# lcp29/trimesh-ray-optix

Hardware: AMD Instinct MI355X
Metric: Mrays/s closest-hit, 1M-tri mesh, 1024^2 ray batch (higher is better)
Workload: dtype f32; 1 GPU; C5(i): icosphere(8)+displacement seed 0, 1310720 tris; 1024x1024 pinhole rays per GPU; intersects_closest (stream_compaction=False); rays_per_gpu=1048576, rays_total=1048576, triangles=1310720, parallelism=ray-sharded x1, BVH replicated, warmup_steps_done=360, bvh_depth=30, bvh_bytes=104857568

## Files before the change

trimesh-ray-optix_amd/csrc/kernels_direct.inc:

```
template <bool C, bool DEEP = false> struct tr_word { typedef uint64_t T; };
template <> struct tr_word<true, false> { typedef uint32_t T; };

constexpr bool TR_STREAM_QN = true;
template <int Q> constexpr bool TR_STREAM_COLD = Q != TR_Q_CLOSEST;
template <int Q, int K, bool STATS, bool COMPACT = false, bool UNI = false, bool DEEP = false>
__device__ __forceinline__ void wave_traverse(const tr_bvh_view& b, tr_ray& r, bool go,
                                              tr_result& res, tr_topk<K>& top, tr_counters* cnt,
                                              const tr_ring ring) {
    tr_result_init(res);
    if (Q == TR_Q_LOCATION) top.init();
    typedef typename tr_word<COMPACT, DEEP>::T W;
    tr_state_t<W> fs;
    tr_state_init(fs);
    if (!go) fs.node = -1;
    while (!tr_done(fs)) {
        tr_fused_step<Q, K, STATS, COMPACT, W, UNI, true>(b, r, fs, res, top, cnt, ring);
        TR_CONVERGE();
        tr_fused_step<Q, K, STATS, COMPACT, W, UNI, false>(b, r, fs, res, top, cnt, ring);
        TR_CONVERGE();
    }
}

constexpr uint32_t TR_STEAL_EVERY = 3u;
constexpr uint32_t TR_STEAL_EARLY = 4u;
constexpr int TR_STEAL_IDLE = 1;
__device__ __forceinline__ int lane_rank(unsigned long long mask) {
    return (int)__builtin_amdgcn_mbcnt_hi((unsigned)(mask >> 32), __builtin_amdgcn_mbcnt_lo((unsigned)mask, 0u));
}

template <int Q, bool STATS, bool COMPACT, bool DEEP = false, bool QN = false>
__device__ __forceinline__ bool wave_traverse_steal(const tr_bvh_view& b, tr_ray& r, bool go,
                                                    tr_result& res, tr_counters* cnt,
                                                    const tr_ring ring, int32_t* wl, int lane,
                                                    uint32_t steal_min, bool& lost) {
    constexpr bool PLAIN = QN;
    typedef typename std::conditional<PLAIN, tr_plaina_w, typename tr_word<COMPACT, DEEP>::T>::type W;
    lost = false;
    tr_result_init(res);
    tr_topk<1> top;
    tr_state_t<W> fs;
    const tr_aring ar = tr_aring_of(ring);
    (void)ar;
    if constexpr (PLAIN) tr_state_init(fs, tr_addr_start(ring));
    else tr_state_init(fs);
    if (!go) fs.node = -1;
    auto trip_step = [&](auto test_tag) {
        constexpr bool TEST = decltype(test_tag)::value;
        if (!tr_done(fs)) tr_fused_step<Q, 1, STATS, COMPACT, W, false, TEST, QN>(b, r, fs, res, top, cnt, ring);
    };
    int owner = lane;
    bool split = false;
    uint32_t trip = 0;
    if (steal_min & 0x8000u) {
        steal_min &= 0x7fffu;
        const unsigned long long act = __ballot(go);
        if (act != 0ull) {
            const int l0 = (int)__builtin_ctzll(act);
            const float ax = __shfl(r.dx, l0), ay = __shfl(r.dy, l0), az = __shfl(r.dz, l0);
            const float bx = __shfl(r.ox, l0) - r.ox, by = __shfl(r.oy, l0) - r.oy, bz = __shfl(r.oz, l0) - r.oz;
            const float dd = ax * r.dx + ay * r.dy + az * r.dz;
            const float n0 = ax * ax + ay * ay + az * az, n1 = r.dx * r.dx + r.dy * r.dy + r.dz * r.dz;
            const float ex = 65535.f * b.frame.scale[0], ey = 65535.f * b.frame.scale[1], ez = 65535.f * b.frame.scale[2];
            const bool alike = dd > 0.f && dd * dd >= 0.998f * n0 * n1 && bx * bx + by * by + bz * bz <= 1e-4f * (ex * ex + ey * ey + ez * ez);
            if (4 * __popcll(__ballot(go && alike)) < 3 * __popcll(act) && steal_min > TR_STEAL_EARLY) steal_min = TR_STEAL_EARLY;
        }
    }
    typedef __attribute__((address_space(3))) volatile int32_t lds_i32;
    typedef __attribute__((address_space(3))) volatile unsigned long long lds_u64;
    lds_i32* const lw = (lds_i32*)wl;
    lds_i32* const list = lw;
    lds_i32* const xnode = lw + 64;
    lds_i32* const xdepth = lw + 128;
    int32_t* const xflags = wl + 128;
    if constexpr (PLAIN) xdepth[lane] = 0;
    constexpr int ACC = 192;
    int32_t* sum = wl + ACC;
    unsigned long long* keys = reinterpret_cast<unsigned long long*>(wl + ACC);
    lds_i32* const vsum = lw + ACC;
    lds_u64* const vkeys = (lds_u64*)(lw + ACC);
    lds_i32* const vslots = lw + ACC + 128;
    auto deposit = [&]() {
        if constexpr (PLAIN) {
            if (tr_addr_lost(fs.sa)) atomicOr(&xflags[owner], 0x100);
        }
        if (Q == TR_Q_COUNT) {
            if (res.count) atomicAdd(&sum[owner], res.count);
        } else if (Q == TR_Q_ANY) {
            if (res.best_face >= 0) vsum[owner] = 1;
        } else {
            const bool have = res.best_slot >= 0;
            const unsigned long long key = ((unsigned long long)(__float_as_uint(res.best_t) & 0x7fffffffu) << 32) |
                                           (unsigned)res.best_face;
            if (have) atomicMin(&keys[owner], key);
            __builtin_amdgcn_wave_barrier();
            if (have && vkeys[owner] == key) vslots[owner] = res.best_slot;
        }
    };
    uint32_t k0 = 0;
    if constexpr (PLAIN) {
        bool l0 = false, l1 = false;
        int32_t c0 = 0, c1 = 0;
        while (trip < steal_min) {
            l0 = false; l1 = false;
            if (fs.node >= 0) tr_descent_step<Q, STATS, COMPACT>(b, r, fs, res, cnt, ring, l0, l1, c0, c1);
            TR_CONVERGE();
            trip++;
            if (TR_WAVE_ANY(l0 || l1) || !TR_WAVE_ANY(fs.node >= 0)) break;
        }
        fs.p0 = l0 ? ~c0 : (l1 ? ~c1 : -1);
        fs.p1 = (l0 && l1) ? ~c1 : -1;
        if (trip & 1u) {
            trip_step(std::false_type{});
            TR_CONVERGE();
            trip++;
        }
        k0 = trip == 0u ? 0u : ((trip - 1u) & TR_STEAL_EVERY) + 1u;
        trip -= k0;
    }
    for (;;) {
#pragma unroll 1
        for (uint32_t k = k0; k <= TR_STEAL_EVERY; k += 2) {
            trip_step(std::true_type{});
            TR_CONVERGE();
            trip_step(std::false_type{});
            TR_CONVERGE();
        }
        k0 = 0;
        trip += (TR_STEAL_EVERY / 2u + 1u) * 2u;
        if (split) {
            if (Q == TR_Q_ANY) {
                if (res.best_face >= 0) vsum[owner] = 1;
                __builtin_amdgcn_wave_barrier();
                if (vsum[owner] != 0 && !tr_done(fs)) { fs.node = -1; fs.p0 = -1; fs.p1 = -1; fs.p2 = -1; }
            } else if (Q == TR_Q_CLOSEST || Q == TR_Q_FIRST) {
                const bool have = res.best_slot >= 0;
                const unsigned long long mine = ((unsigned long long)(__float_as_uint(res.best_t) & 0x7fffffffu) << 32) |
                                                (unsigned)(res.best_face < 0 ? 0x7fffffff : res.best_face);
                if (have) atomicMin(&keys[owner], mine);
                __builtin_amdgcn_wave_barrier();
                const unsigned long long k = vkeys[owner];
                if (have && k == mine) vslots[owner] = res.best_slot;
                if (k < mine) {
                    tr_set_best_t(res, __uint_as_float((unsigned)(k >> 32)));
                    res.best_face = (int32_t)(unsigned)k;
                    res.best_slot = -1;
                }
            }
        }
        const bool done = tr_done(fs);
        const unsigned long long idle = __ballot(done);
        if (idle == ~0ull) break;
        if (__popcll(idle) >= TR_STEAL_IDLE && trip >= steal_min) {
            uint32_t bot = 0;
            bool has_far;
            if constexpr (PLAIN) {
                bot = (uint32_t)xdepth[lane] & 0xffu;
                has_far = tr_addr_can_give(ar, fs.sa, bot);
            } else {
                has_far = (fs.trail & fs.owned) != 0;
            }
            const bool can_give = !done && has_far;
            const unsigned long long donors = __ballot(can_give);
            const int ni = __popcll(idle), nd = __popcll(donors);
            const int np = ni < nd ? ni : nd;
            if (np > 0) {
                if (!split) {
                    if (Q == TR_Q_COUNT || Q == TR_Q_ANY) vsum[lane] = 0;
                    else vkeys[lane] = ~0ull;
                    split = true;
                    __builtin_amdgcn_wave_barrier();
                }
                const int drank = lane_rank(donors), irank = lane_rank(idle);
                const bool give = can_give && drank < np;
                int gnode = 0, gdepth = 0;
                (void)gdepth;
                if constexpr (PLAIN) {
                    if (give) {
                        gnode = tr_addr_give(ar, fs.sa, bot);
                        list[drank] = lane; xnode[lane] = gnode;
                        atomicAdd(&xflags[lane], 1);
                    }
                } else if (give) {
                    uint32_t j;
                    gnode = tr_ring_get(ring, tr_bottom_slot<W>(fs.trail, fs.owned, j));
                    gdepth = (int32_t)(j + 1);
                    list[drank] = lane; xnode[lane] = gnode; xdepth[lane] = gdepth;
                    fs.trail &= ~(W(1) << j);
                }
                __builtin_amdgcn_wave_barrier();
                const bool take = done && irank < np;
                const int src = take ? list[irank] : lane;
                if (take) {
                    deposit();
                    tr_result_init(res);
                }
                r.ox = __shfl(r.ox, src); r.oy = __shfl(r.oy, src); r.oz = __shfl(r.oz, src);
                r.dx = __shfl(r.dx, src); r.dy = __shfl(r.dy, src); r.dz = __shfl(r.dz, src);
                r.ix = __shfl(r.ix, src); r.iy = __shfl(r.iy, src); r.iz = __shfl(r.iz, src);
                r.kd = __shfl(r.kd, src);
                r.sel_n = (uint32_t)__shfl((int)r.sel_n, src); r.sel_f = (uint32_t)__shfl((int)r.sel_f, src); r.sel_z = (uint32_t)__shfl((int)r.sel_z, src);
                if constexpr (QN) {
                    r.qax = __shfl(r.qax, src); r.qay = __shfl(r.qay, src); r.qaz = __shfl(r.qaz, src);
                    r.qnx = __shfl(r.qnx, src); r.qny = __shfl(r.qny, src); r.qnz = __shfl(r.qnz, src);
                    r.qfx = __shfl(r.qfx, src); r.qfy = __shfl(r.qfy, src); r.qfz = __shfl(r.qfz, src);
                    r.qaz2 = r.qaz;
                }
                const int own2 = __shfl(owner, src);
                const float bt = __shfl(res.best_t, src);
                if (take) {
                    owner = own2;
                    if constexpr (PLAIN) {
                        tr_state_init(fs, tr_addr_bottom(ar, fs.sa));
                        atomicAnd(&xflags[lane], 0x100);
                    } else {
                        tr_state_init(fs);
                        fs.depth = (uint32_t)xdepth[src];
                    }
                    fs.node = xnode[src];
                    tr_set_best_t(res, bt);
                }
                __builtin_amdgcn_wave_barrier();
            }
        }
    }
    if (split) {
        deposit();
        __builtin_amdgcn_wave_barrier();
        if (Q == TR_Q_COUNT) {
            res.count = vsum[lane];
        } else if (Q == TR_Q_ANY) {
            res.best_face = vsum[lane] ? 0 : -1;
        } else {
            const unsigned long long k = vkeys[lane];
            tr_result_init(res);
            if (k != ~0ull) {
                tr_set_best_t(res, __uint_as_float((unsigned)(k >> 32)));
                res.best_face = (int32_t)(unsigned)k;
                res.best_slot = vslots[lane];
            }
        }
        if constexpr (PLAIN) lost = (xdepth[lane] & 0x100) != 0;
    } else if constexpr (PLAIN) {
        lost = tr_addr_lost(fs.sa);
    }
    return split;
}

template <int Q, bool STATS, bool COMPACT = false, bool UNI = false, bool DEEP = false>
__device__ __forceinline__ void process_ray(const tr_bvh_view& b, const RayFetch& rf,
                                            const QueryOut& out, int64_t i, bool in_range,
                                            tr_counters* cnt, const tr_ring ring) {
    float o[3] = {0.f, 0.f, 0.f}, d[3] = {0.f, 0.f, 0.f};
    if (in_range) fetch_ray(rf, i, o, d);
    tr_ray r;
    const bool valid = tr_ray_setup_a(r, b.frame, o[0], o[1], o[2], d[0], d[1], d[2]) && in_range;
    tr_result res;
    if (Q == TR_Q_LOCATION) {
        tr_topk<0> top;
        top.ent = out.hits + (in_range ? i : 0) * out.cap;
        top.tris = b.tris;
        top.cap = out.cap;
        if (b.num_tris >= 2) {
            wave_traverse<Q, 0, STATS, COMPACT, UNI, DEEP>(b, r, valid, res, top, cnt, ring);
        } else {
            top.init();
            brute_one<Q>(b, r, valid, res);
            if (res.count) top.insert(res.best_t, res.best_face, 0);
        }
    } else {
        tr_topk<1> top;
        if (b.num_tris >= 2) wave_traverse<Q, 1, STATS, COMPACT, UNI, DEEP>(b, r, valid, res, top, cnt, ring);
        else brute_one<Q>(b, r, valid, res);
    }
    if (in_range) write_result<Q>(b, out, i, r, res);
}

template <int Q>
__device__ __attribute__((noinline)) tr_result retraverse_lost(const tr_node* nodes, const tr_link* links, const tr_tri* tris,
                                                               float b0, float b1, float b2, float s0, float s1, float s2,
                                                               float ox, float oy, float oz, float dx, float dy, float dz,
                                                               float best_t, int32_t best_face, int32_t best_slot) {
    tr_bvh_view v;
    v.nodes = nodes; v.links = links; v.tris = tris; v.num_tris = 2; v.qnodes = nullptr; v.frame_dev = nullptr;
    v.frame.base[0] = b0; v.frame.base[1] = b1; v.frame.base[2] = b2;
    v.frame.scale[0] = s0; v.frame.scale[1] = s1; v.frame.scale[2] = s2;
    tr_result res;
    res.best_t = best_t; res.best_face = best_face; res.best_slot = best_slot; res.count = 0;
    tr_ray r;
    if (tr_ray_setup_a(r, v.frame, ox, oy, oz, dx, dy, dz)) {
        tr_topk<1> top;
        tr_counters* nc = nullptr;
        tr_traverse_more<Q, 1, false>(v, r, res, top, nc);
    }
    return res;
}

template <int Q, bool STATS, bool COMPACT, bool DEEP = false, bool QN = false>
__device__ __forceinline__ void process_ray_steal(const tr_bvh_view& b, const RayFetch& rf,
                                                  const QueryOut& out, int64_t i, bool in_range,
                                                  tr_counters* cnt, const tr_ring ring, int32_t* wl,
                                                  uint32_t steal_min) {
    float o[3] = {0.f, 0.f, 0.f}, d[3] = {0.f, 0.f, 0.f};
    if (in_range) fetch_ray(rf, i, o, d);
    tr_ray r;
    const bool valid = tr_ray_setup_q(r, b.frame, o[0], o[1], o[2], d[0], d[1], d[2]) && in_range;
    tr_result res;
    bool split = false, lost = false;
    if (b.num_tris >= 2) split = wave_traverse_steal<Q, STATS, COMPACT, DEEP, QN>(b, r, valid, res, cnt, ring, wl, (int)(threadIdx.x & 63), steal_min, lost);
    else brute_one<Q>(b, r, valid, res);
    if (split && in_range) {
        fetch_ray(rf, i, o, d);
        tr_ray_setup_a(r, b.frame, o[0], o[1], o[2], d[0], d[1], d[2]);
    }
    if constexpr (QN) {
        lost = lost && valid;
        if (__builtin_expect(TR_WAVE_ANY(lost), 0)) {
            if (lost) {
                fetch_ray(rf, i, o, d);
                res = retraverse_lost<Q>(b.nodes, b.links, b.tris, b.frame.base[0], b.frame.base[1], b.frame.base[2],
                                         b.frame.scale[0], b.frame.scale[1], b.frame.scale[2], o[0], o[1], o[2], d[0], d[1], d[2],
                                         res.best_t, res.best_face, res.best_slot);
            }
        }
    }
    if (in_range) write_result<Q>(b, out, i, r, res);
}

template <int Q, int K, bool STATS, bool COMPACT, bool DEEP = false>
__device__ __forceinline__ void wave_traverse_unordered(const tr_bvh_view& b, tr_ray& r, bool go,
                                                        tr_result& res, tr_topk<K>& top, tr_counters* cnt,
                                                        const tr_ring ring, const tr_leafq lq, int leaf_min) {
    typedef typename tr_word<COMPACT, DEEP>::T W;
    tr_result_init(res);
    if (Q == TR_Q_LOCATION) top.init();
    tr_ustate_t<W> st;
    tr_ustate_init(st);
    if (!go) st.node = -1;
    for (;;) {
        const bool can_node = tr_ucan_node(st);
        const unsigned long long mn = __ballot(can_node), ml = __ballot(st.nq > 0);
        if ((mn | ml) == 0ull) break;
        const bool parked = st.node >= 0 && !can_node;
        const bool leaf_phase = mn == 0ull || __ballot(parked) != 0ull || (int)__popcll(ml) >= (int)leaf_min;
        tr_unord_step<Q, K, STATS, COMPACT, W>(b, r, can_node, leaf_phase, st, res, top, cnt, ring, lq);
        TR_CONVERGE();
    }
}

template <int Q, bool STATS, bool COMPACT, bool DEEP = false>
__device__ __forceinline__ int wave_count_unordered_steal(const tr_bvh_view& b, tr_ray& r, bool go, tr_counters* cnt,
                                                          const tr_ring ring, const tr_leafq lq, int leaf_min,
                                                          int lane, uint32_t steal_min) {
    typedef typename tr_word<COMPACT, DEEP>::T W;
    tr_result res;
    tr_result_init(res);
    tr_topk<1> top;
    tr_ustate_t<W> st;
    tr_ustate_init(st);
    if (!go) st.node = -1;
    int owner = lane;
    int acc = 0;
    uint32_t trip = 0;
    auto hand_in = [&](bool want) {
        unsigned long long m = __ballot(want && res.count != 0);
        while (m != 0ull) {
            const int t = (int)__builtin_ctzll(m);
            const int o = __builtin_amdgcn_readlane(owner, t), c = __builtin_amdgcn_readlane(res.count, t);
            if (lane == o) acc += c;
            m &= m - 1ull;
        }
        if (want) res.count = 0;
    };
    for (;;) {
        bool live = true;
#pragma unroll 1
        for (int k = 0; k < 4 && live; k++) {
            const bool can_node = tr_ucan_node(st);
            const unsigned long long mn = __ballot(can_node), ml = __ballot(st.nq > 0);
            live = (mn | ml) != 0ull;
            if (live) {
                const bool parked = st.node >= 0 && !can_node;
                const bool leaf_phase = mn == 0ull || __ballot(parked) != 0ull || (int)__popcll(ml) >= (int)leaf_min;
                tr_unord_step<Q, 1, STATS, COMPACT, W>(b, r, can_node, leaf_phase, st, res, top, cnt, ring, lq);
            }
            TR_CONVERGE();
        }
        trip += 4;
        const bool done = tr_udone(st);
        const unsigned long long idle = __ballot(done);
        if (idle == ~0ull) break;
        if (idle == 0ull) continue;
        const W cand = st.trail & st.owned;
        const bool can_give = !done && cand != 0 && trip >= steal_min;
        const unsigned long long donors = __ballot(can_give);
        const int ni = __popcll(idle), nd = __popcll(donors);
        const int np = ni < nd ? ni : nd;
        if (np == 0) continue;
        const int drank = lane_rank(donors), irank = lane_rank(idle);
        const bool give = can_give && drank < np;
        const bool take = done && irank < np;
        const unsigned long long givers = __ballot(give);
        const int tgt = give ? drank : 63 - lane_rank(~givers);
        const int list = __builtin_amdgcn_ds_permute(tgt << 2, lane);
        const int pick = __shfl(list, irank & 63);
        const int src = take ? pick : lane;
// ... 409 lines not shown
```

trimesh-ray-optix_amd/csrc/tr_bvh.h:

```cpp
#pragma once
#include <type_traits>
#include "tr_math.h"
#include "../../include/triro_hip.h"

struct alignas(16) tr_f4 {
    float x, y, z, w;
};
struct alignas(16) tr_i4 {
    int32_t x, y, z, w;
};

struct alignas(64) tr_node {
    float box0[6];
    float box1[6];
    int32_t c0, c1;
    int32_t parent;
    int32_t sibling;
};
static_assert(sizeof(tr_node) == 64, "node must be 64 B");
TR_HD void tr_node_set_box(float* box, const float* lo, const float* hi) {
    box[0] = lo[0]; box[1] = lo[1]; box[2] = lo[2]; box[3] = hi[2]; box[4] = hi[0]; box[5] = hi[1];
}

struct alignas(8) tr_link {
// ... 516 lines not shown
        uint32_t j = 0;
        int32_t far = -1;
        if (tr_pop_far(ring, st.trail, st.owned, j, far)) {
            st.node = far;
        } else {
            int32_t node = st.node;
            uint32_t depth = st.depth;
            while (depth > j + 1) {
                node = parent;
                const tr_link l = b.links[node];
                parent = l.parent; sibling = l.sibling;
                depth--;
                if (STATS) cnt->climbs++;
            }
            st.node = sibling;
        }
        st.depth = j + 1;
    }
}

template <int Q, int K, bool STATS>
TR_HD void tr_leaf_step(const tr_bvh_view& b, const tr_ray& r, tr_state& st, tr_result& res,
                        tr_topk<K>& top, tr_counters* cnt) {
    const int32_t q0 = st.p0, q1 = st.p1;
    tr_counters* nc = nullptr;
    const bool any1 = TR_WAVE_ANY(q1 >= 0);
    const tr_tri t0 = tr_load_tri<false>(b, q0 >= 0 ? q0 : 0, nc);
    tr_tri t1 = t0;
    if (any1) t1 = tr_load_tri<false>(b, q1 >= 0 ? q1 : 0, nc);
    if (STATS && q0 >= 0) cnt->tris++;
    bool fin = tr_fold_leaf<Q, K>(q0 >= 0, r, t0, q0, res, top, st.pe);
    fin = tr_drain_exact<Q, K>(b, r, st.pe, res, top) || fin;
    if (any1) {
        const bool live = q1 >= 0 && !fin;
        if (STATS && live) cnt->tris++;
        fin = tr_fold_leaf<Q, K>(live, r, t1, q1, res, top, st.pe) || fin;
        fin = tr_drain_exact<Q, K>(b, r, st.pe, res, top) || fin;
    }
    st.p0 = -1; st.p1 = -1;
    if (Q == TR_Q_ANY && fin) st.node = -1;
}

TR_HD void tr_qnode_slabs_contract(const tr_ray& r, const tr_qframe& f, const tr_i4& w0, const tr_i4& w1,
                                   float& tn0, float& tf0, float& tn1, float& tf1) {
    const uint32_t q0 = (uint32_t)w0.x, q1 = (uint32_t)w0.y, q2 = (uint32_t)w0.z, q3 = (uint32_t)w0.w;
    const uint32_t q4 = (uint32_t)w1.x, q5 = (uint32_t)w1.y;
    const float sx = f.scale[0], sy = f.scale[1], sz = f.scale[2], bx = f.base[0], by = f.base[1], bz = f.base[2];
    tr_slab(r, tr_qdecode(q0 & 0xffffu, sx, bx), tr_qdecode(q0 >> 16, sy, by), tr_qdecode(q1 & 0xffffu, sz, bz),
            tr_qdecode(q2 & 0xffffu, sx, bx), tr_qdecode(q2 >> 16, sy, by), tr_qdecode(q1 >> 16, sz, bz), tn0, tf0);
    tr_slab(r, tr_qdecode(q3 & 0xffffu, sx, bx), tr_qdecode(q3 >> 16, sy, by), tr_qdecode(q4 & 0xffffu, sz, bz),
            tr_qdecode(q5 & 0xffffu, sx, bx), tr_qdecode(q5 >> 16, sy, by), tr_qdecode(q4 >> 16, sz, bz), tn1, tf1);
}

TR_HD void tr_qnode_slabs(const tr_ray& r, const tr_qframe& f, const tr_i4& w0, const tr_i4& w1,
                          float& tn0, float& tf0, float& tn1, float& tf1) {
#if defined(__HIP_DEVICE_COMPILE__)
    const uint32_t q0 = (uint32_t)w0.x, q1 = (uint32_t)w0.y, q2 = (uint32_t)w0.z, q3 = (uint32_t)w0.w;
    const uint32_t q4 = (uint32_t)w1.x, q5 = (uint32_t)w1.y;
    typedef float tr_v2 __attribute__((ext_vector_type(2)));
    const tr_v2 axy = {r.qax, r.qay}, azz = {r.qaz, r.qaz2};
    const tr_v2 nxy = {r.qnx, r.qny}, fxy = {r.qfx, r.qfy}, bz = {r.qnz, r.qfz};
#define TR_UNPK(w) tr_v2{(float)((w) & 0xffffu), (float)((w) >> 16)}
    {
        const uint32_t pn = __builtin_amdgcn_perm(q2, q0, r.sel_n), pf = __builtin_amdgcn_perm(q2, q0, r.sel_f);
        const uint32_t zz = __builtin_amdgcn_perm(q1, q1, r.sel_z);
        const tr_v2 a = __builtin_elementwise_fma(TR_UNPK(pn), axy, nxy);
        const tr_v2 c = __builtin_elementwise_fma(TR_UNPK(pf), axy, fxy);
        const tr_v2 b = __builtin_elementwise_fma(TR_UNPK(zz), azz, bz);
        tn0 = fmaxf(fmaxf(a.x, a.y), b.x);
        tf0 = fminf(fminf(c.x, c.y), b.y);
    }
    {
        const uint32_t pn = __builtin_amdgcn_perm(q5, q3, r.sel_n), pf = __builtin_amdgcn_perm(q5, q3, r.sel_f);
        const uint32_t zz = __builtin_amdgcn_perm(q4, q4, r.sel_z);
        const tr_v2 a = __builtin_elementwise_fma(TR_UNPK(pn), axy, nxy);
        const tr_v2 c = __builtin_elementwise_fma(TR_UNPK(pf), axy, fxy);
        const tr_v2 b = __builtin_elementwise_fma(TR_UNPK(zz), azz, bz);
        tn1 = fmaxf(fmaxf(a.x, a.y), b.x);
        tf1 = fminf(fminf(c.x, c.y), b.y);
    }
#undef TR_UNPK
#else
    (void)f;
    const bool nx = r.ix < 0.f, ny = r.iy < 0.f, nz = r.iz < 0.f;
    const uint32_t q[6] = {(uint32_t)w0.x, (uint32_t)w0.y, (uint32_t)w0.z, (uint32_t)w0.w, (uint32_t)w1.x, (uint32_t)w1.y};
    float tn[2], tf[2];
    for (int c = 0; c < 2; c++) {
        const uint32_t lox = q[3 * c] & 0xffffu, loy = q[3 * c] >> 16, loz = q[3 * c + 1] & 0xffffu;
        const uint32_t hiz = q[3 * c + 1] >> 16, hix = q[3 * c + 2] & 0xffffu, hiy = q[3 * c + 2] >> 16;
        const float ax = fmaf((float)(nx ? hix : lox), r.qax, r.qnx), ay = fmaf((float)(ny ? hiy : loy), r.qay, r.qny);
        const float az = fmaf((float)(nz ? hiz : loz), r.qaz, r.qnz);
        const float cx = fmaf((float)(nx ? lox : hix), r.qax, r.qfx), cy = fmaf((float)(ny ? loy : hiy), r.qay, r.qfy);
        const float cz = fmaf((float)(nz ? loz : hiz), r.qaz, r.qfz);
        tn[c] = fmaxf(fmaxf(ax, ay), az);
        tf[c] = fminf(fminf(cx, cy), cz);
    }
    tn0 = tn[0]; tf0 = tf[0]; tn1 = tn[1]; tf1 = tf[1];
#endif
}

template <bool STATS>
TR_HD int32_t tr_climb(const tr_bvh_view& b, int32_t node, uint32_t depth, uint32_t j, tr_counters* cnt) {
    tr_link l = b.links[node];
    if (STATS) cnt->climbs++;
    while (depth > j + 1) {
        node = l.parent;
        l = b.links[node];
        depth--;
        if (STATS) cnt->climbs++;
    }
    return l.sibling;
}

struct tr_rec_f { tr_f4 n0, n1, n2, n3; };
struct tr_rec_q { tr_i4 w0, w1; };
TR_HD void tr_rec_slabs(const tr_bvh_view&, const tr_ray& r, const tr_rec_f& n, float& tn0, float& tf0, float& tn1, float& tf1) {
    tr_node_slabs(r, n.n0, n.n1, n.n2, tn0, tf0, tn1, tf1);
}
TR_HD void tr_rec_slabs(const tr_bvh_view& b, const tr_ray& r, const tr_rec_q& n, float& tn0, float& tf0, float& tn1, float& tf1) {
    tr_qnode_slabs(r, b.frame, n.w0, n.w1, tn0, tf0, tn1, tf1);
}
TR_HD void tr_rec_children(const tr_rec_f& n, int32_t& c0, int32_t& c1) {
    union { float f; int32_t i; } u0, u1;
    u0.f = n.n3.x; u1.f = n.n3.y; c0 = u0.i; c1 = u1.i;
}
TR_HD void tr_rec_children(const tr_rec_q& n, int32_t& c0, int32_t& c1) { c0 = n.w1.z; c1 = n.w1.w; }
TR_HD void tr_rec_links(const tr_rec_f& n, int32_t& parent, int32_t& sibling) {
    union { float f; int32_t i; } u2, u3;
    u2.f = n.n3.z; u3.f = n.n3.w; parent = u2.i; sibling = u3.i;
}
TR_HD void tr_rec_links(const tr_rec_q&, int32_t& parent, int32_t& sibling) { parent = -1; sibling = -1; }

template <int Q, int K, bool STATS, bool COMPACT, typename W, bool TEST, bool COLD, typename REC>
TR_HD void tr_fused_body(const tr_bvh_view& b, const tr_ray& r, tr_state_t<W>& st, tr_result& res,
                         tr_topk<K>& top, tr_counters* cnt, const tr_ring ring, const bool has_node,
                         const REC& rec) {
    if (STATS && has_node) cnt->nodes++;
    bool fin = false;
    const int32_t q0 = st.p0;
    if (TEST && TR_WAVE_ANY(q0 >= 0)) {
        tr_counters* nc = nullptr;
        const tr_tri t0 = tr_load_tri<false, COMPACT>(b, q0 >= 0 ? q0 : 0, nc);
        const bool live = q0 >= 0;
        if (STATS && live) cnt->tris++;
        fin = tr_fold_leaf<Q, K>(live, r, t0, q0, res, top, st.pe);
    }
    if (Q == TR_Q_ANY && fin) { st.node = -1; st.p1 = -1; st.p2 = -1; }
    float tn0, tf0, tn1, tf1;
    tr_rec_slabs(b, r, rec, tn0, tf0, tn1, tf1);
    int32_t c0, c1, parent, sibling;
    tr_rec_children(rec, c0, c1);
    tr_rec_links(rec, parent, sibling);
    const float lim = tr_cull_limit<Q>(res);
    const bool go = has_node && st.node >= 0;
    bool h0 = tr_slab_hit(tn0, tf0, lim) && go;
    bool h1 = tr_slab_hit(tn1, tf1, lim) && go;
    if (!TEST) {
        const bool l0 = h0 && c0 < 0, l1 = h1 && c1 < 0;
        h0 = h0 && c0 >= 0;
        h1 = h1 && c1 >= 0;
        if (go) {
            const bool hb = st.p0 >= 0, two = l0 && l1;
            const int32_t xi = l0 ? ~c0 : (l1 ? ~c1 : -1);
            st.p2 = (hb && two) ? ~c1 : -1;
            st.p1 = hb ? xi : (two ? ~c1 : -1);
            st.p0 = hb ? st.p0 : xi;
        }
    } else {
        const bool l0 = h0 && c0 < 0;
        const bool wait = st.p2 >= 0;
        const bool l1 = (h1 && c1 < 0) || wait;
        h0 = h0 && c0 >= 0;
        h1 = h1 && c1 >= 0;
        const int32_t i1 = wait ? st.p2 : ~c1;
        const bool hb = st.p1 >= 0, two = l0 && l1;
        const int32_t xi = l0 ? ~c0 : (l1 ? i1 : -1);
        st.p0 = hb ? st.p1 : xi;
        st.p1 = hb ? xi : (two ? i1 : -1);
        st.p2 = (hb && two) ? i1 : -1;
    }
    if constexpr (std::is_same<W, tr_plain_w>::value) {
        if (go) {
            const bool both = h0 && h1;
            const bool swap = (both && tn1 < tn0) || !h0;
            if (both) tr_plain_push(ring, st.sp, swap ? c0 : c1);
            st.node = swap ? c1 : c0;
            if (!(h0 || h1)) st.node = tr_plain_pop(ring, st.sp);
        }
    } else if constexpr (std::is_same<W, tr_plaina_w>::value) {
        if (go) {
            const tr_aring ar = tr_aring_of(ring);
            const bool both = h0 && h1;
            const bool swap = (both && tn1 < tn0) || !h0;
            if (both) tr_addr_push(ar, st.sa, swap ? c0 : c1);
            st.node = swap ? c1 : c0;
            if (!(h0 || h1)) st.node = tr_addr_pop(ar, st.sa);
        }
    } else if (go) {
        if (h0 || h1) {
            const bool both = h0 && h1;
            const bool swap = (both && tn1 < tn0) || !h0;
            if (both) {
                tr_push_far(ring, st.trail, st.owned, st.depth, swap ? c0 : c1);
                st.trail |= (W(1) << st.depth);
            }
            st.node = swap ? c1 : c0;
            st.depth++;
        } else if (st.trail == 0) {
            st.node = -1;
        } else {
            uint32_t j = 0;
            int32_t far = -1;
            if (!tr_pop_far(ring, st.trail, st.owned, j, far)) {
                if constexpr (std::is_same<REC, tr_rec_f>::value) {
                    int32_t node = st.node;
                    uint32_t depth = st.depth;
                    while (depth > j + 1) {
                        node = parent;
                        const tr_link l = b.links[node];
                        parent = l.parent; sibling = l.sibling;
                        depth--;
                        if (STATS) cnt->climbs++;
                    }
                    far = sibling;
                } else {
                    far = tr_climb<STATS>(b, st.node, st.depth, j, cnt);
                }
            }
            st.node = far;
            st.depth = j + 1;
        }
    }
    if (TEST) {
        if (tr_drain_exact<Q, K, COMPACT, COLD>(b, r, st.pe, res, top) && Q == TR_Q_ANY) { st.node = -1; st.p0 = -1; st.p1 = -1; st.p2 = -1; }
        st.pe = -1;
    }
}


template <int Q, int K, bool STATS, bool COMPACT = false, typename W = uint64_t, bool UNI = false, bool TEST = true,
          bool QN = false, bool COLD = true>
TR_HD void tr_fused_step(const tr_bvh_view& b, const tr_ray& r, tr_state_t<W>& st, tr_result& res,
                         tr_topk<K>& top, tr_counters* cnt, const tr_ring ring) {
    const int32_t room = TEST ? st.p2 : st.p1;
    const bool has_node = st.node >= 0 && room < 0;
#if defined(__HIP_DEVICE_COMPILE__)
    if (UNI) {
        const unsigned long long m = __ballot(has_node);
        if (m != 0ull) {
            const int32_t nu = __builtin_amdgcn_readlane(st.node, (int)__builtin_ctzll(m));
            if (__ballot(has_node && st.node != nu) == 0ull) {
                if constexpr (QN) {
                    typedef const __attribute__((address_space(4))) tr_i4* tr_ci4p;
                    const tr_ci4p sp = (tr_ci4p)(unsigned long long)tr_qnode_ptr<COMPACT>(b, nu);
                    const tr_rec_q rec = {sp[0], sp[1]};
                    tr_fused_body<Q, K, STATS, COMPACT, W, TEST, COLD>(b, r, st, res, top, cnt, ring, has_node, rec);
                } else {
                    typedef const __attribute__((address_space(4))) tr_f4* tr_cf4p;
                    const tr_cf4p sp = (tr_cf4p)(unsigned long long)tr_node_ptr<COMPACT>(b, nu);
                    const tr_rec_f rec = {sp[0], sp[1], sp[2], sp[3]};
                    tr_fused_body<Q, K, STATS, COMPACT, W, TEST, COLD>(b, r, st, res, top, cnt, ring, has_node, rec);
                }
                return;
            }
        }
    }
#endif
    const int32_t nidx = st.node & ~(st.node >> 31) & (room >> 31);
    if constexpr (QN) {
        const tr_i4* np = tr_qnode_ptr<COMPACT>(b, nidx);
        const tr_rec_q rec = {np[0], np[1]};
        tr_fused_body<Q, K, STATS, COMPACT, W, TEST, COLD>(b, r, st, res, top, cnt, ring, has_node, rec);
    } else {
        const tr_f4* np = tr_node_ptr<COMPACT>(b, nidx);
        const tr_rec_f rec = {np[0], np[1], np[2], np[3]};
        tr_fused_body<Q, K, STATS, COMPACT, W, TEST, COLD>(b, r, st, res, top, cnt, ring, has_node, rec);
    }
}

template <int Q, bool STATS, bool COMPACT>
TR_HD void tr_descent_step(const tr_bvh_view& b, const tr_ray& r, tr_astate& st, const tr_result& res, tr_counters* cnt,
                           const tr_ring ring, bool& l0, bool& l1, int32_t& c0, int32_t& c1) {
    const tr_i4* np = tr_qnode_ptr<COMPACT>(b, st.node);
    const tr_rec_q rec = {np[0], np[1]};
    if (STATS) cnt->nodes++;
    float tn0, tf0, tn1, tf1;
    tr_rec_slabs(b, r, rec, tn0, tf0, tn1, tf1);
    tr_rec_children(rec, c0, c1);
    const float lim = tr_cull_limit<Q>(res);
    bool h0 = tr_slab_hit(tn0, tf0, lim);
    bool h1 = tr_slab_hit(tn1, tf1, lim);
    l0 = h0 && c0 < 0;
    l1 = h1 && c1 < 0;
    h0 = h0 && c0 >= 0;
    h1 = h1 && c1 >= 0;
    const tr_aring ar = tr_aring_of(ring);
    const bool both = h0 && h1;
    const bool swap = (both && tn1 < tn0) || !h0;
    if (both) tr_addr_push(ar, st.sa, swap ? c0 : c1);
    st.node = swap ? c1 : c0;
    if (!(h0 || h1)) st.node = tr_addr_pop(ar, st.sa);
}


constexpr int TR_LEAFQ = 6;
struct tr_leafq {
    int32_t* base;
    int32_t stride;
};

template <typename W>
struct tr_ustate_t {
    int32_t node;
    uint32_t depth;
    W trail, owned;
    int32_t nq;
    int32_t pe;
};

template <typename W>
TR_HD void tr_ustate_init(tr_ustate_t<W>& st) { st.node = 0; st.depth = 0; st.trail = 0; st.owned = 0; st.nq = 0; st.pe = -1; }
template <typename W>
TR_HD bool tr_udone(const tr_ustate_t<W>& st) { return st.node < 0 && st.nq == 0 && st.pe < 0; }
template <typename W>
TR_HD bool tr_ucan_node(const tr_ustate_t<W>& st) { return st.node >= 0 && st.nq <= TR_LEAFQ - 2; }

template <int Q, int K, bool STATS, bool COMPACT, typename W>
TR_HD void tr_unord_step(const tr_bvh_view& b, const tr_ray& r, bool go_node, bool leaf_phase,
                         tr_ustate_t<W>& st, tr_result& res, tr_topk<K>& top, tr_counters* cnt,
                         const tr_ring ring, const tr_leafq lq) {
    const int32_t nidx = go_node ? st.node : 0;
    const tr_i4* np = COMPACT ? reinterpret_cast<const tr_i4*>(reinterpret_cast<const char*>(b.qnodes) + ((uint32_t)nidx << 5))
                              : reinterpret_cast<const tr_i4*>(b.qnodes + nidx);
    const tr_i4 w0 = np[0], w1 = np[1];
    if (STATS && go_node) cnt->nodes++;
    bool fin = false;
    if (leaf_phase) {
        const bool gl = st.nq > 0;
        int32_t slot = 0;
        if (gl) { st.nq--; slot = lq.base[st.nq * lq.stride]; }
        tr_counters* nc = nullptr;
        const tr_tri t = tr_load_tri<false, COMPACT>(b, slot, nc);
        if (STATS && gl) cnt->tris++;
        fin = tr_fold_leaf<Q, K>(gl, r, t, slot, res, top, st.pe);
    }
    if (Q == TR_Q_ANY && fin) { st.node = -1; st.nq = 0; }
    const bool go = go_node && !fin;
    float tn0, tf0, tn1, tf1;
    tr_qnode_slabs(r, b.frame, w0, w1, tn0, tf0, tn1, tf1);
    const int32_t c0 = w1.z, c1 = w1.w;
    bool h0 = tr_slab_hit(tn0, tf0, TR_TLIM) && go;
    bool h1 = tr_slab_hit(tn1, tf1, TR_TLIM) && go;
    if (h0 && c0 < 0) { lq.base[st.nq * lq.stride] = ~c0; st.nq++; h0 = false; }
    if (h1 && c1 < 0) { lq.base[st.nq * lq.stride] = ~c1; st.nq++; h1 = false; }
    if (go) {
        if (h0 || h1) {
            const bool both = h0 && h1;
            const bool swap = (Q == TR_Q_ANY) ? ((both && tn1 < tn0) || !h0) : !h0;
            if (both) {
                st.trail |= (W(1) << st.depth);
                if (ring.base) {
                    const uint32_t slot = st.depth & (TR_RING - 1);
                    tr_ring_put(ring, slot, swap ? c0 : c1);
                    st.owned = (st.owned & ~(tr_ring_mask(W(0)) << slot)) | (W(1) << st.depth);
                }
            }
            st.node = swap ? c1 : c0;
            st.depth++;
        } else if (st.trail == 0) {
            st.node = -1;
        } else {
            const uint32_t j = tr_top_bit(st.trail);
            st.trail &= ~(W(1) << j);
            if (ring.base && ((st.owned >> j) & W(1))) st.node = tr_ring_get(ring, j & (TR_RING - 1));
            else st.node = tr_climb<STATS>(b, st.node, st.depth, j, cnt);
            st.depth = j + 1;
        }
    }
    if (leaf_phase) {
        if (tr_drain_exact<Q, K, COMPACT>(b, r, st.pe, res, top) && Q == TR_Q_ANY) { st.node = -1; st.nq = 0; }
        st.pe = -1;
    }
}

template <int Q, int K, bool STATS>
TR_HD void tr_traverse_unordered(const tr_bvh_view& b, const tr_ray& r, bool valid, tr_result& res,
                                 tr_topk<K>& top, tr_counters* cnt, const tr_ring ring, const tr_leafq lq) {
    tr_result_init(res);
    if (Q == TR_Q_LOCATION) top.init();
    if (!valid || b.num_tris < 2) return;
    tr_ustate_t<uint64_t> st;
    tr_ustate_init(st);
    while (!tr_udone(st)) {
        const bool cn = tr_ucan_node(st);
        tr_unord_step<Q, K, STATS, false, uint64_t>(b, r, cn, !cn, st, res, top, cnt, ring, lq);
        TR_CONVERGE();
    }
}

template <int Q, int K, bool STATS>
TR_HD void tr_traverse_more(const tr_bvh_view& b, const tr_ray& r, tr_result& res, tr_topk<K>& top, tr_counters* cnt) {
    if (Q == TR_Q_ANY && res.best_face >= 0) return;
    tr_state st;
    tr_state_init(st);
    while (!tr_done(st)) {
        if (tr_pending(st)) tr_leaf_step<Q, K, STATS>(b, r, st, res, top, cnt);
        else tr_node_step<Q, STATS>(b, r, st, res, cnt, tr_ring{nullptr, 0});
        TR_CONVERGE();
    }
}

template <int Q, int K, bool STATS>
TR_HD void tr_traverse(const tr_bvh_view& b, const tr_ray& r, bool valid, tr_result& res,
                       tr_topk<K>& top, tr_counters* cnt, const tr_ring ring = tr_ring{nullptr, 0}) {
    tr_result_init(res);
    if (Q == TR_Q_LOCATION) top.init();
    if (!valid || b.num_tris < 2) return;
    tr_state st;
    tr_state_init(st);
    while (!tr_done(st)) {
        if (tr_pending(st)) tr_leaf_step<Q, K, STATS>(b, r, st, res, top, cnt);
        else tr_node_step<Q, STATS>(b, r, st, res, cnt, ring);
        TR_CONVERGE();
    }
}
```

Measured before the change: 7869 Mrays/s.

## Add wave-uniform scalar-load descent for coherent top of BVH traversal

```diff
diff --git a/trimesh-ray-optix_amd/csrc/kernels_direct.inc b/trimesh-ray-optix_amd/csrc/kernels_direct.inc
--- a/trimesh-ray-optix_amd/csrc/kernels_direct.inc
+++ b/trimesh-ray-optix_amd/csrc/kernels_direct.inc
@@ -100,7 +100,46 @@
     if constexpr (PLAIN) {
         bool l0 = false, l1 = false;
         int32_t c0 = 0, c1 = 0;
-        while (trip < steal_min) {
+        bool stop = false;
+        {
+            const unsigned long long act = __ballot(go);
+            if (act != 0ull && trip < steal_min) {
+                const int first = (int)__builtin_ctzll(act);
+                const uint32_t sn = (uint32_t)__builtin_amdgcn_readlane((int)r.sel_n, first);
+                const uint32_t sf = (uint32_t)__builtin_amdgcn_readlane((int)r.sel_f, first);
+                const uint32_t sz = (uint32_t)__builtin_amdgcn_readlane((int)r.sel_z, first);
+                if (__ballot(go && (r.sel_n != sn || r.sel_f != sf || r.sel_z != sz)) == 0ull) {
+                    const tr_uoctant oct = tr_uniform_octant(sn, sz);
+                    int32_t nu = 0;
+                    tr_uwave u;
+                    bool more;
+#pragma unroll 1
+                    do {
+                        typedef const __attribute__((address_space(4))) int32_t* tr_ci32p;
+                        const tr_ci32p sp = (tr_ci32p)(unsigned long long)tr_qnode_ptr<COMPACT>(b, nu);
+                        tr_i4 w0, w1;
+                        w0.x = sp[0]; w0.y = sp[1]; w0.z = sp[2]; w0.w = sp[3];
+                        w1.x = sp[4]; w1.y = sp[5]; w1.z = sp[6]; w1.w = sp[7];
+                        bool a0, a1, lt;
+                        tr_uniform_test<Q>(r, w0, w1, oct, res, a0, a1, lt);
+                        if (STATS && go) cnt->nodes++;
+                        u = tr_uniform_wave(act, __builtin_amdgcn_ballot_w64(a0), __builtin_amdgcn_ballot_w64(a1),
+                                            __builtin_amdgcn_ballot_w64(lt), w1.z, w1.w);
+                        c0 = w1.z; c1 = w1.w;
+                        if (tr_lane_in(u.both, lane)) tr_addr_push(ar, fs.sa, tr_lane_in(u.sw, lane) ? c0 : c1);
+                        TR_CONVERGE();
+                        trip++;
+                        more = ((u.l0 | u.l1 | u.pop) == 0ull) & ((u.sw == 0ull) | (u.sw == act)) & (trip < steal_min);
+                        nu = u.sw != 0ull ? c1 : c0;
+                    } while (more);
+                    l0 = tr_lane_in(u.l0, lane); l1 = tr_lane_in(u.l1, lane);
+                    if (go) fs.node = tr_lane_in(u.sw, lane) ? c1 : c0;
+                    if (tr_lane_in(u.pop, lane)) fs.node = tr_addr_pop(ar, fs.sa);
+                    stop = (u.l0 | u.l1) != 0ull || !TR_WAVE_ANY(fs.node >= 0);
+                }
+            }
+        }
+        if (!stop) while (trip < steal_min) {
             l0 = false; l1 = false;
             if (fs.node >= 0) tr_descent_step<Q, STATS, COMPACT>(b, r, fs, res, cnt, ring, l0, l1, c0, c1);
             TR_CONVERGE();
diff --git a/trimesh-ray-optix_amd/csrc/tr_bvh.h b/trimesh-ray-optix_amd/csrc/tr_bvh.h
--- a/trimesh-ray-optix_amd/csrc/tr_bvh.h
+++ b/trimesh-ray-optix_amd/csrc/tr_bvh.h
@@ -842,6 +842,68 @@
     if (!(h0 || h1)) st.node = tr_addr_pop(ar, st.sa);
 }
 
+struct tr_uoctant {
+    uint32_t mxy;
+    uint32_t she, shf;
+};
+TR_HD tr_uoctant tr_uniform_octant(uint32_t sel_n, uint32_t sel_z) {
+    const bool nx = (sel_n & 0x0400u) != 0u, ny = (sel_n & 0x04000000u) != 0u, nz = (sel_z & 2u) != 0u;
+    return tr_uoctant{(nx ? 0xffffu : 0u) | (ny ? 0xffff0000u : 0u), nz ? 16u : 0u, nz ? 0u : 16u};
+}
+template <int Q>
+TR_HD void tr_uniform_test(const tr_ray& r, const tr_i4& w0, const tr_i4& w1, const tr_uoctant& oct, const tr_result& res,
+                           bool& a0, bool& a1, bool& lt) {
+    const uint32_t q[6] = {(uint32_t)w0.x, (uint32_t)w0.y, (uint32_t)w0.z, (uint32_t)w0.w, (uint32_t)w1.x, (uint32_t)w1.y};
+    float tn[2], tf[2];
+#pragma unroll
+    for (int c = 0; c < 2; c++) {
+        const uint32_t t = (q[3 * c] ^ q[3 * c + 2]) & oct.mxy;
+        const uint32_t e = q[3 * c] ^ t, f = q[3 * c + 2] ^ t, z = q[3 * c + 1];
+        const float ex = (float)(e & 0xffffu), ey = (float)(e >> 16), ez = (float)((z >> oct.she) & 0xffffu);
+        const float fx = (float)(f & 0xffffu), fy = (float)(f >> 16), fz = (float)((z >> oct.shf) & 0xffffu);
+#if defined(__HIP_DEVICE_COMPILE__)
+        typedef float tr_v2 __attribute__((ext_vector_type(2)));
+        const tr_v2 a = __builtin_elementwise_fma(tr_v2{ex, ey}, tr_v2{r.qax, r.qay}, tr_v2{r.qnx, r.qny});
+        const tr_v2 b = __builtin_elementwise_fma(tr_v2{fx, fy}, tr_v2{r.qax, r.qay}, tr_v2{r.qfx, r.qfy});
+        const tr_v2 d = __builtin_elementwise_fma(tr_v2{ez, fz}, tr_v2{r.qaz, r.qaz2}, tr_v2{r.qnz, r.qfz});
+        tn[c] = fmaxf(fmaxf(a.x, a.y), d.x);
+        tf[c] = fminf(fminf(b.x, b.y), d.y);
+#else
+        tn[c] = fmaxf(fmaxf(fmaf(ex, r.qax, r.qnx), fmaf(ey, r.qay, r.qny)), fmaf(ez, r.qaz, r.qnz));
+        tf[c] = fminf(fminf(fmaf(fx, r.qax, r.qfx), fmaf(fy, r.qay, r.qfy)), fmaf(fz, r.qaz, r.qfz));
+#endif
+    }
+    const float lim = tr_cull_limit<Q>(res);
+    a0 = tr_slab_hit(tn[0], tf[0], lim);
+    a1 = tr_slab_hit(tn[1], tf[1], lim);
+    lt = tn[1] < tn[0];
+}
+struct tr_uwave {
+    uint64_t l0, l1;
+    uint64_t both;
+    uint64_t sw;
+    uint64_t pop;
+};
+TR_HD tr_uwave tr_uniform_wave(uint64_t act, uint64_t a0, uint64_t a1, uint64_t lt, int32_t c0, int32_t c1) {
+    const uint64_t m0 = a0 & act, m1 = a1 & act;
+    const uint64_t h0 = c0 >= 0 ? m0 : 0ull, h1 = c1 >= 0 ? m1 : 0ull;
+    tr_uwave u;
+    u.l0 = m0 ^ h0;
+    u.l1 = m1 ^ h1;
+    u.both = h0 & h1;
+    u.sw = ((u.both & lt) | ~h0) & act;
+    u.pop = act & ~(h0 | h1);
+    return u;
+}
+TR_HD bool tr_lane_in(uint64_t mask, int lane) {
+#if defined(__HIP_DEVICE_COMPILE__)
+    (void)lane;
+    return __builtin_amdgcn_inverse_ballot_w64(mask);
+#else
+    return ((mask >> lane) & 1ull) != 0ull;
+#endif
+}
+
 
 constexpr int TR_LEAFQ = 6;
 struct tr_leafq {
```

New measurement: 8136 Mrays/s (median of 6 runs). 3.4% higher.
